# nju-websoft/OpenEA

Hardware: AMD Instinct MI355X
Metric: training triples/sec (k=10 truncated negatives + limited loss + Adagrad) (higher is better)
Workload: dtype f32; 1 GPU; BootEA/AlignE translational step, EN-FR-100K-V1 shape (synthetic), dim=100, GLOBAL batch=20000 positives (weak scaling: 20000 per GPU x 1 GPU), k=10, truncated eps=0.98; the same workload at every N (; global_batch=20000, entities=200000, parallelism=single

## Files before the change

openea_amd/csrc/step_plan.hip:

```cpp
#include <string.h>

#include <rocprim/rocprim.hpp>

#include <algorithm>

#include "common.h"
#include "step_plan.h"

namespace oea {

static size_t al256(size_t x) { return (x + 255) / 256 * 256; }
static int bits_for(uint64_t max_value) { int b = 1; while (b < 64 && (max_value >> b) != 0) ++b; return b; }

size_t step_plan_layout(int64_t n_total, int32_t steps, int64_t max_batch, int64_t n_ent, int32_t ld, void *base, StepPlanView *v) {
    const size_t m = (size_t)std::max<int64_t>(2 * n_total, 1);
    size_t off = 0;
    char *b = static_cast<char *>(base);
    auto take = [&](size_t bytes) { size_t o = off; off += al256(bytes); return b ? b + o : nullptr; };
    StepPlanView w{};
    w.keys_a = (uint64_t *)take(8 * m);
    w.keys_b = (uint64_t *)take(8 * m);
    w.vals_a = (uint32_t *)take(4 * m);
    w.vals_b = (uint32_t *)take(4 * m);
    w.ukeys = (uint64_t *)take(8 * m);
    w.ucount = (uint32_t *)take(4 * (m + 1));
    w.uoff = (uint32_t *)take(4 * (m + 1));
    w.n_unique = (int32_t *)take(4);
    w.step_first = (int32_t *)take(4 * ((size_t)steps + 1));
    w.pflags = (uint32_t *)take(4 * (size_t)std::max<int64_t>(n_total, 1));
    w.recs = (uint4 *)take(16 * m);
    w.inplan = (uint8_t *)take((size_t)std::max<int32_t>(steps, 1) * (size_t)n_ent);
    w.contrib = (float *)take(sizeof(float) * 2 * (size_t)std::max<int64_t>(max_batch, 1) * (size_t)ld);
    size_t t1 = 0, t2 = 0, t3 = 0;
    (void)rocprim::radix_sort_pairs(nullptr, t1, (const uint64_t *)nullptr, (uint64_t *)nullptr, (const uint32_t *)nullptr,
                                    (uint32_t *)nullptr, m, 0, 64, (hipStream_t)0);
    (void)rocprim::run_length_encode(nullptr, t2, (const uint64_t *)nullptr, m, (uint64_t *)nullptr, (uint32_t *)nullptr,
                                     (int32_t *)nullptr, (hipStream_t)0);
    (void)rocprim::exclusive_scan(nullptr, t3, (const uint32_t *)nullptr, (uint32_t *)nullptr, 0u, m + 1, rocprim::plus<uint32_t>(),
                                  (hipStream_t)0);
    const size_t n1 = (size_t)std::max<int64_t>(n_total, 1);
    w.temp_bytes = std::max(std::max(t1, std::max(t2, t3)), al256(4 * n1)) + 256;
    w.temp = take(w.temp_bytes);
    w.rel_order = (uint32_t *)take(4 * n1);
    w.row_bits = bits_for((uint64_t)std::max<int64_t>(n_ent - 1, 1));
    if (v) *v = w;
    return off;
}

namespace {

__global__ void plan_emit_kernel(const int32_t *__restrict__ pos_all, const int32_t *__restrict__ neg_all, int k,
                                 const int64_t *__restrict__ offsets, int steps, int64_t n_total, int row_bits,
                                 uint64_t *__restrict__ keys, uint32_t *__restrict__ vals) {
    const int64_t p = (int64_t)blockIdx.x * blockDim.x + threadIdx.x;
    if (p >= n_total) return;
    int lo = 0, hi = steps;
    while (hi - lo > 1) {
        const int mid = (lo + hi) >> 1;
        if (offsets[mid] <= p) lo = mid; else hi = mid;
    }
    const uint32_t pl = (uint32_t)(p - offsets[lo]);
    const int h = pos_all[3 * p], r = pos_all[3 * p + 1], t = pos_all[3 * p + 2];
    unsigned bad = 0, xh = 0, xt = 0;
    const int32_t *ng = neg_all + p * k * 3;
    for (int j = 0; j < k; ++j) {
        const unsigned a = (unsigned)(ng[3 * j] ^ h), b = (unsigned)(ng[3 * j + 2] ^ t), c = (unsigned)(ng[3 * j + 1] ^ r);
        bad |= c | min(a, b);
        xh |= a;
        xt |= b;
    }
    if (bad | min(xh, xt)) {
        keys[2 * p] = keys[2 * p + 1] = (uint64_t)steps << row_bits;
        vals[2 * p] = vals[2 * p + 1] = 0u;
        return;
    }
    const bool tails = xh == 0;
    const uint64_t sk = (uint64_t)lo << row_bits;
    keys[2 * p] = sk | (uint64_t)(uint32_t)h;
    vals[2 * p] = 2u * pl + (tails ? 0u : 1u);
    keys[2 * p + 1] = sk | (uint64_t)(uint32_t)t;
    vals[2 * p + 1] = 0x80000000u | (2u * pl + (tails ? 1u : 0u));
}

constexpr int kRelSortWaves = 8, kRelDigitBits = 10, kRelBins = 1 << kRelDigitBits, kRelAhead = 8;
__global__ __launch_bounds__(kRelSortWaves * 64) void plan_rel_order_kernel(const int32_t *__restrict__ pos_all, const int64_t *__restrict__ offsets,
                                                                            uint32_t *__restrict__ tmp, uint32_t *__restrict__ rel_order) {
    __shared__ uint32_t hist[kRelSortWaves][kRelBins];
    __shared__ uint32_t dbase[kRelBins];
    __shared__ uint32_t wsum[kRelSortWaves];
    __shared__ uint32_t rmax;
    const int64_t first = offsets[blockIdx.x];
    const uint32_t n = (uint32_t)(offsets[blockIdx.x + 1] - first);
    if (n == 0) return;
    const int32_t *rel = pos_all + 3 * first + 1;
    const uint32_t t = threadIdx.x, lane = t & 63u, w = t >> 6;
    const uint32_t slice = (n + kRelSortWaves - 1) / kRelSortWaves, c0 = min(w * slice, n), c1 = min(c0 + slice, n);
    const uint32_t groups = (c1 - c0 + 63u) / 64u;
    if (t == 0) rmax = 0u;
    int passes = 1;
    uint32_t *src = nullptr, *dst = nullptr;
    for (int pass = 0; pass < passes; ++pass) {
        const int shift = pass * kRelDigitBits;
        for (uint32_t i = t; i < kRelSortWaves * kRelBins; i += blockDim.x) (&hist[0][0])[i] = 0u;
        __syncthreads();
        uint32_t m = 0u;
        for (uint32_t g0 = 0; g0 < groups; g0 += kRelAhead) {
            uint32_t r[kRelAhead];
#pragma unroll
            for (int u = 0; u < kRelAhead; ++u) {
                const uint32_t i = c0 + (g0 + u) * 64u + lane;
                r[u] = i < c1 ? (uint32_t)rel[3 * (int64_t)(src ? src[i] : i)] : 0xffffffffu;
            }
#pragma unroll
            for (int u = 0; u < kRelAhead; ++u)
                if (c0 + (g0 + u) * 64u + lane < c1) {
                    m = max(m, r[u]);
                    atomicAdd(&hist[w][(r[u] >> shift) & (kRelBins - 1)], 1u);
                }
        }
        if (pass == 0) {
            for (int o = 32; o > 0; o >>= 1) m = max(m, (uint32_t)__shfl_xor((int)m, o));
            if (lane == 0) atomicMax(&rmax, m);
        }
        __syncthreads();
        if (pass == 0) {
            while (passes * kRelDigitBits < 32 && (rmax >> (passes * kRelDigitBits)) != 0u) ++passes;
            dst = (passes & 1) ? rel_order + first : tmp + first;
        }
        constexpr int DPT = kRelBins / (kRelSortWaves * 64);
        uint32_t tot[DPT], mine = 0u;
#pragma unroll
        for (int j = 0; j < DPT; ++j) {
            uint32_t run = 0u;
            for (int x = 0; x < kRelSortWaves; ++x) { const uint32_t c = hist[x][t * DPT + j]; hist[x][t * DPT + j] = run; run += c; }
            tot[j] = run;
            mine += run;
        }
        uint32_t inc = mine;
        for (int o = 1; o < 64; o <<= 1) { const uint32_t y = (uint32_t)__shfl_up((int)inc, o); if (lane >= (uint32_t)o) inc += y; }
        if (lane == 63u) wsum[w] = inc;
        __syncthreads();
        uint32_t before = inc - mine;
        for (uint32_t x = 0; x < w; ++x) before += wsum[x];
#pragma unroll
        for (int j = 0; j < DPT; ++j) { dbase[t * DPT + j] = before; before += tot[j]; }
        __syncthreads();
        for (uint32_t g0 = 0; g0 < groups; g0 += kRelAhead) {
            uint32_t idx[kRelAhead], dg[kRelAhead];
#pragma unroll
            for (int u = 0; u < kRelAhead; ++u) {
                const uint32_t i = c0 + (g0 + u) * 64u + lane;
                idx[u] = i < c1 ? (src ? src[i] : i) : 0u;
                dg[u] = i < c1 ? ((uint32_t)rel[3 * (int64_t)idx[u]] >> shift) & (kRelBins - 1) : 0u;
            }
#pragma unroll
            for (int u = 0; u < kRelAhead; ++u) {
                const bool on = c0 + (g0 + u) * 64u + lane < c1;
                const uint32_t d = dg[u];
                unsigned long long same = __ballot(on);
#pragma unroll
                for (int b = 0; b < kRelDigitBits; ++b) {
                    const unsigned long long has = __ballot(on && ((d >> b) & 1u));
                    same &= ((d >> b) & 1u) ? has : ~has;
                }
                if (on) {
                    const uint32_t rank = (uint32_t)__popcll(same & ((1ull << lane) - 1ull));
                    const uint32_t slot = hist[w][d] + dbase[d] + rank;
                    dst[slot] = idx[u];
                    __builtin_amdgcn_wave_barrier();
                    if (rank == 0u) hist[w][d] += (uint32_t)__popcll(same);
                }
                __builtin_amdgcn_wave_barrier();
            }
        }
        __threadfence_block();
        __syncthreads();
        src = dst;
        dst = (dst == tmp + first) ? rel_order + first : tmp + first;
    }
}

__global__ void plan_step_first_kernel(const uint64_t *__restrict__ ukeys, const int32_t *__restrict__ n_unique, int steps, int row_bits,
                                       int32_t *__restrict__ step_first) {
    const int s = blockIdx.x * blockDim.x + threadIdx.x;
    if (s > steps) return;
    const uint64_t key = (uint64_t)s << row_bits;
    int lo = 0, hi = *n_unique;
    while (lo < hi) {
        const int mid = (lo + hi) >> 1;
        if (ukeys[mid] < key) lo = mid + 1; else hi = mid;
    }
    step_first[s] = lo;
}

__global__ void plan_records_kernel(const uint64_t *__restrict__ ukeys, const uint32_t *__restrict__ uoff, const uint32_t *__restrict__ vals,
                                    const int32_t *__restrict__ n_unique, int steps, int row_bits, int64_t n_ent, uint4 *__restrict__ recs,
                                    uint8_t *__restrict__ inplan) {
    const int nu = *n_unique;
    for (int64_t i = (int64_t)blockIdx.x * blockDim.x + threadIdx.x; i < nu; i += (int64_t)gridDim.x * blockDim.x) {
        const uint64_t key = ukeys[i];
        const uint32_t row = (uint32_t)(key & (((uint64_t)1 << row_bits) - 1)), e0 = uoff[i], cnt = uoff[i + 1] - e0;
        recs[i] = make_uint4(row, e0, cnt, vals[e0]);
        const int64_t step = (int64_t)(key >> row_bits);
        if (step < steps && cnt <= kPlanHubEntries) inplan[step * n_ent + row] = 1;
    }
}

__global__ void plan_hub_kernel(const uint64_t *__restrict__ keys, const uint32_t *__restrict__ vals, int64_t m,
                                const int64_t *__restrict__ offsets, int steps, int row_bits, uint32_t *__restrict__ pflags) {
    const int64_t e = (int64_t)blockIdx.x * blockDim.x + threadIdx.x;
    if (e >= m) return;
    const uint64_t key = keys[e];
    const int64_t step = (int64_t)(key >> row_bits);
    if (step >= steps) return;
    int left = 0, right = 0;
    while (left < (int)kPlanHubEntries && e - left - 1 >= 0 && keys[e - left - 1] == key) ++left;
    while (left + right < (int)kPlanHubEntries && e + right + 1 < m && keys[e + right + 1] == key) ++right;
    if (left + right < (int)kPlanHubEntries) return;
    const uint32_t v = vals[e];
    atomicOr(&pflags[offsets[step] + ((v & 0x7fffffffu) >> 1)], (v >> 31) ? 2u : 1u);
}

__device__ __forceinline__ uint32_t mix32(uint32_t x) {
    x ^= x >> 16; x *= 0x7feb352du; x ^= x >> 15; x *= 0x846ca68bu; x ^= x >> 16;
    return x;
}
__device__ __forceinline__ uint32_t feistel_perm(uint32_t i, uint32_t n, int lbits, int rbits, const uint32_t (&key)[6]) {
    const uint32_t lmask = (1u << lbits) - 1u, rmask = (1u << rbits) - 1u;
    uint32_t x = i;
    do {
        uint32_t l = x >> rbits, r = x & rmask;
#pragma unroll
        for (int q = 0; q < 6; q += 2) {
            l = (l ^ mix32(r ^ key[q])) & lmask;
            r = (r ^ mix32(l ^ key[q + 1])) & rmask;
        }
        x = (l << rbits) | r;
    } while (x >= n);
    return x;
}
__global__ void layout_perm_kernel(const int32_t *__restrict__ triples, int64_t n1, int64_t n2, const int64_t *__restrict__ slot, int64_t n_slots,
                                   uint32_t k0, uint32_t k1, uint32_t epoch, int32_t *__restrict__ dall) {
    const int64_t j = (int64_t)blockIdx.x * blockDim.x + threadIdx.x;
    if (j >= n_slots) return;
    const int64_t sj = slot[j];
    const bool second = sj >= n1;
    const uint32_t n = (uint32_t)(second ? n2 : n1), i = (uint32_t)(second ? sj - n1 : sj);
    int bits = 1;
    while (bits < 32 && (1ull << bits) < (unsigned long long)n) ++bits;
    if (bits < 2) bits = 2;
    const int rbits = bits / 2, lbits = bits - rbits;
    const uint4 wa = philox4x32_10(epoch, second ? 1u : 0u, 0x5eedu, 0u, k0, k1), wb = philox4x32_10(epoch, second ? 1u : 0u, 0x5eedu, 1u, k0, k1);
    const uint32_t key[6] = {wa.x, wa.y, wa.z, wa.w, wb.x, wb.y};
    const int64_t src = (int64_t)feistel_perm(i, n, lbits, rbits, key) + (second ? n1 : 0);
    dall[3 * j] = triples[3 * src]; dall[3 * j + 1] = triples[3 * src + 1]; dall[3 * j + 2] = triples[3 * src + 2];
}

}
}

extern "C" {

size_t oea_step_plan_bytes(int64_t n_total, int32_t steps, int64_t max_batch, int64_t n_ent, int32_t ld) {
    if (n_total < 0 || steps < 0 || max_batch < 0 || n_ent <= 0 || ld <= 0) return 0;
    return oea::step_plan_layout(n_total, steps, max_batch, n_ent, ld, nullptr, nullptr);
}

int oea_step_plan_offsets(int64_t n_total, int32_t steps, int64_t max_batch, int64_t n_ent, int32_t ld, int64_t *out) {
    OEA_REQUIRE(out && n_total >= 0 && steps >= 0 && n_ent > 0 && ld > 0, "arguments");
    oea::StepPlanView v;
    char *base = reinterpret_cast<char *>(4096);
    const size_t total = oea::step_plan_layout(n_total, steps, max_batch, n_ent, ld, base, &v);
    out[0] = (char *)v.vals_b - base; out[1] = (char *)v.ukeys - base; out[2] = (char *)v.uoff - base;
    out[3] = (char *)v.n_unique - base; out[4] = (char *)v.step_first - base; out[5] = (char *)v.contrib - base;
    out[6] = v.row_bits; out[7] = (int64_t)total; out[8] = (char *)v.pflags - base;
    return OEA_OK;
}

int oea_step_plan_rel_order_offset(int64_t n_total, int32_t steps, int64_t max_batch, int64_t n_ent, int32_t ld, int64_t *out) {
    OEA_REQUIRE(out && n_total >= 0 && steps >= 0 && n_ent > 0 && ld > 0, "arguments");
    oea::StepPlanView v;
    char *base = reinterpret_cast<char *>(4096);
    (void)oea::step_plan_layout(n_total, steps, max_batch, n_ent, ld, base, &v);
    *out = (char *)v.rel_order - base;
    return OEA_OK;
}

size_t oea_epoch_layout_bytes(int64_t n) {
    return n < 0 ? 0 : 256;
}

int oea_epoch_layout(const int32_t *triples, int64_t n1, int64_t n2, const int64_t *slot, int64_t n_slots, uint64_t seed, uint32_t epoch,
                     int32_t *dall, void *workspace, size_t ws_bytes, void *stream) {
    OEA_REQUIRE(triples && (slot || n_slots == 0) && (dall || n_slots == 0), "null pointer");
    OEA_REQUIRE(n1 >= 0 && n2 >= 0 && n_slots >= 0 && n1 < ((int64_t)1 << 32) && n2 < ((int64_t)1 << 32), "sizes");
    (void)workspace; (void)ws_bytes;
    if (n1 + n2 == 0 || n_slots == 0) return OEA_OK;
    hipStream_t st = oea::as_stream(stream);
    oea::layout_perm_kernel<<<(unsigned)oea::ceil_div(n_slots, 256), 256, 0, st>>>(triples, n1, n2, slot, n_slots, (uint32_t)seed,
                                                                                   (uint32_t)(seed >> 32), epoch, dall);
    OEA_CHECK_HIP(hipGetLastError());
    return OEA_OK;
}

int oea_step_plan_build(const int32_t *pos_all, const int32_t *neg_all, int32_t k, const int64_t *offsets_dev, int64_t n_total,
                        int32_t steps, int64_t max_batch, int64_t n_ent, int32_t ld, void *plan, size_t plan_bytes, void *stream) {
    OEA_REQUIRE(pos_all && offsets_dev && plan && (neg_all || k == 0), "null pointer");
    OEA_REQUIRE(n_total >= 0 && steps >= 1 && k >= 0 && n_ent > 0 && ld > 0, "sizes");
    OEA_REQUIRE(2 * n_total < ((int64_t)1 << 31) && 2 * max_batch < ((int64_t)1 << 31), "entries and slots are 31-bit");
    oea::StepPlanView v;
    const size_t need = oea::step_plan_layout(n_total, steps, max_batch, n_ent, ld, plan, &v);
    OEA_REQUIRE(plan_bytes >= need, "plan workspace smaller than oea_step_plan_bytes");
    hipStream_t st = oea::as_stream(stream);
    const size_t m = (size_t)(2 * n_total);
    if (m == 0) {
        OEA_CHECK_HIP(hipMemsetAsync(v.n_unique, 0, sizeof(int32_t), st));
        OEA_CHECK_HIP(hipMemsetAsync(v.step_first, 0, sizeof(int32_t) * ((size_t)steps + 1), st));
        return OEA_OK;
    }
    oea::plan_rel_order_kernel<<<(unsigned)steps, oea::kRelSortWaves * 64, 0, st>>>(pos_all, offsets_dev, (uint32_t *)v.temp, v.rel_order);
    oea::plan_emit_kernel<<<(unsigned)oea::ceil_div(n_total, 256), 256, 0, st>>>(pos_all, neg_all, k, offsets_dev, steps, n_total, v.row_bits,
                                                                                 v.keys_a, v.vals_a);
    const int end_bit = std::min(64, v.row_bits + oea::bits_for((uint64_t)steps));
    size_t tb = v.temp_bytes;
    OEA_CHECK_HIP(rocprim::radix_sort_pairs(v.temp, tb, (const uint64_t *)v.keys_a, v.keys_b, (const uint32_t *)v.vals_a, v.vals_b, m, 0,
                                            (unsigned)end_bit, st));
    OEA_CHECK_HIP(hipMemsetAsync(v.ucount, 0, sizeof(uint32_t) * (m + 1), st));
    tb = v.temp_bytes;
    OEA_CHECK_HIP(rocprim::run_length_encode(v.temp, tb, (const uint64_t *)v.keys_b, m, v.ukeys, v.ucount, v.n_unique, st));
    tb = v.temp_bytes;
    OEA_CHECK_HIP(rocprim::exclusive_scan(v.temp, tb, (const uint32_t *)v.ucount, v.uoff, 0u, m + 1, rocprim::plus<uint32_t>(), st));
    oea::plan_step_first_kernel<<<(unsigned)oea::ceil_div(steps + 1, 256), 256, 0, st>>>(v.ukeys, v.n_unique, steps, v.row_bits, v.step_first);
    OEA_CHECK_HIP(hipMemsetAsync(v.pflags, 0, sizeof(uint32_t) * (size_t)n_total, st));
    OEA_CHECK_HIP(hipMemsetAsync(v.inplan, 0, (size_t)steps * (size_t)n_ent, st));
    oea::plan_records_kernel<<<(unsigned)std::min<int64_t>(oea::ceil_div((int64_t)m, 256), 4096), 256, 0, st>>>(
        v.ukeys, v.uoff, v.vals_b, v.n_unique, steps, v.row_bits, n_ent, v.recs, v.inplan);
    oea::plan_hub_kernel<<<(unsigned)oea::ceil_div((int64_t)m, 256), 256, 0, st>>>(v.keys_b, v.vals_b, (int64_t)m, offsets_dev, steps, v.row_bits,
                                                                                   v.pflags);
    OEA_CHECK_HIP(hipGetLastError());
    return OEA_OK;
}

}
```

Before: 292.7 million triples/s.

## Fuse step-plan post-sort into custom scan kernels and stage emit negatives in LDS

The chain of rocprim run_length_encode, exclusive_scan, step_first binary search, two memsets and the records and hub kernels is replaced by three custom kernels. A per-tile head count kernel (which also zeroes pflags and inplan), a decoupled scan kernel that writes unique keys, offsets, step_first and per-entry group indices, and a finish kernel that emits records and hub flags. The emit kernel stages negatives in shared memory, writes keys and values as vector stores, and skips the step binary search for rejected triples. The relation sort kernel doubles its waves and caches relation ids in 16-bit LDS to avoid re-gathering from global memory on later passes. The aim is fewer launches, fewer memsets and less global traffic in plan building, at the cost of more complex hand-written scan logic.

```diff
diff --git a/openea_amd/csrc/step_plan.hip b/openea_amd/csrc/step_plan.hip
--- a/openea_amd/csrc/step_plan.hip
+++ b/openea_amd/csrc/step_plan.hip
@@ -49,46 +49,65 @@
 
 namespace {
 
-__global__ void plan_emit_kernel(const int32_t *__restrict__ pos_all, const int32_t *__restrict__ neg_all, int k,
-                                 const int64_t *__restrict__ offsets, int steps, int64_t n_total, int row_bits,
-                                 uint64_t *__restrict__ keys, uint32_t *__restrict__ vals) {
-    const int64_t p = (int64_t)blockIdx.x * blockDim.x + threadIdx.x;
+constexpr int kEmitThreads = 256, kEmitStageBytes = 60 * 1024;
+template <bool STAGED>
+__global__ __launch_bounds__(kEmitThreads) void plan_emit_kernel(const int32_t *__restrict__ pos_all, const int32_t *__restrict__ neg_all, int k,
+                                                                 const int64_t *__restrict__ offsets, int steps, int64_t n_total, int row_bits,
+                                                                 uint64_t *__restrict__ keys, uint32_t *__restrict__ vals) {
+    extern __shared__ int4 emit_stage[];
+    const int32_t *stage = reinterpret_cast<const int32_t *>(emit_stage);
+    const int64_t pb = (int64_t)blockIdx.x * kEmitThreads, p = pb + threadIdx.x;
+    const int per = 3 * k;
+    if (STAGED) {
+        const int64_t cnt = min((int64_t)kEmitThreads, n_total - pb) * per, quads = cnt / 4;
+        const int32_t *src = neg_all + pb * per;
+        int32_t *st = reinterpret_cast<int32_t *>(emit_stage);
+        if ((reinterpret_cast<uintptr_t>(src) & 15u) == 0u) {
+            for (int64_t i = threadIdx.x; i < quads; i += kEmitThreads) emit_stage[i] = reinterpret_cast<const int4 *>(src)[i];
+            for (int64_t i = 4 * quads + threadIdx.x; i < cnt; i += kEmitThreads) st[i] = src[i];
+        } else {
+            for (int64_t i = threadIdx.x; i < cnt; i += kEmitThreads) st[i] = src[i];
+        }
+        __syncthreads();
+    }
     if (p >= n_total) return;
-    int lo = 0, hi = steps;
-    while (hi - lo > 1) {
-        const int mid = (lo + hi) >> 1;
-        if (offsets[mid] <= p) lo = mid; else hi = mid;
-    }
-    const uint32_t pl = (uint32_t)(p - offsets[lo]);
     const int h = pos_all[3 * p], r = pos_all[3 * p + 1], t = pos_all[3 * p + 2];
     unsigned bad = 0, xh = 0, xt = 0;
-    const int32_t *ng = neg_all + p * k * 3;
+    const int32_t *ng = STAGED ? stage + (int64_t)threadIdx.x * per : neg_all + p * per;
     for (int j = 0; j < k; ++j) {
         const unsigned a = (unsigned)(ng[3 * j] ^ h), b = (unsigned)(ng[3 * j + 2] ^ t), c = (unsigned)(ng[3 * j + 1] ^ r);
         bad |= c | min(a, b);
         xh |= a;
         xt |= b;
     }
+    ulonglong2 *key2 = reinterpret_cast<ulonglong2 *>(keys) + p;
+    uint2 *val2 = reinterpret_cast<uint2 *>(vals) + p;
     if (bad | min(xh, xt)) {
-        keys[2 * p] = keys[2 * p + 1] = (uint64_t)steps << row_bits;
-        vals[2 * p] = vals[2 * p + 1] = 0u;
+        const uint64_t sentinel = (uint64_t)steps << row_bits;
+        *key2 = make_ulonglong2(sentinel, sentinel);
+        *val2 = make_uint2(0u, 0u);
         return;
     }
+    int lo = 0, hi = steps;
+    while (hi - lo > 1) {
+        const int mid = (lo + hi) >> 1;
+        if (offsets[mid] <= p) lo = mid; else hi = mid;
+    }
+    const uint32_t pl = (uint32_t)(p - offsets[lo]);
     const bool tails = xh == 0;
     const uint64_t sk = (uint64_t)lo << row_bits;
-    keys[2 * p] = sk | (uint64_t)(uint32_t)h;
-    vals[2 * p] = 2u * pl + (tails ? 0u : 1u);
-    keys[2 * p + 1] = sk | (uint64_t)(uint32_t)t;
-    vals[2 * p + 1] = 0x80000000u | (2u * pl + (tails ? 1u : 0u));
-}
-
-constexpr int kRelSortWaves = 8, kRelDigitBits = 10, kRelBins = 1 << kRelDigitBits, kRelAhead = 8;
+    *key2 = make_ulonglong2(sk | (uint64_t)(uint32_t)h, sk | (uint64_t)(uint32_t)t);
+    *val2 = make_uint2(2u * pl + (tails ? 0u : 1u), 0x80000000u | (2u * pl + (tails ? 1u : 0u)));
+}
+
+constexpr int kRelSortWaves = 16, kRelDigitBits = 10, kRelBins = 1 << kRelDigitBits, kRelAhead = 8, kRelCache = 24 * 1024;
 __global__ __launch_bounds__(kRelSortWaves * 64) void plan_rel_order_kernel(const int32_t *__restrict__ pos_all, const int64_t *__restrict__ offsets,
                                                                             uint32_t *__restrict__ tmp, uint32_t *__restrict__ rel_order) {
     __shared__ uint32_t hist[kRelSortWaves][kRelBins];
     __shared__ uint32_t dbase[kRelBins];
     __shared__ uint32_t wsum[kRelSortWaves];
     __shared__ uint32_t rmax;
+    __shared__ uint16_t rcache[kRelCache];
     const int64_t first = offsets[blockIdx.x];
     const uint32_t n = (uint32_t)(offsets[blockIdx.x + 1] - first);
     if (n == 0) return;
@@ -98,6 +117,8 @@
     const uint32_t groups = (c1 - c0 + 63u) / 64u;
     if (t == 0) rmax = 0u;
     int passes = 1;
+    const bool fits = n <= (uint32_t)kRelCache;
+    bool cached = false;
     uint32_t *src = nullptr, *dst = nullptr;
     for (int pass = 0; pass < passes; ++pass) {
         const int shift = pass * kRelDigitBits;
@@ -109,7 +130,15 @@
 #pragma unroll
             for (int u = 0; u < kRelAhead; ++u) {
                 const uint32_t i = c0 + (g0 + u) * 64u + lane;
-                r[u] = i < c1 ? (uint32_t)rel[3 * (int64_t)(src ? src[i] : i)] : 0xffffffffu;
+                if (cached) r[u] = i < c1 ? (uint32_t)rcache[src[i]] : 0xffffffffu;
+                else r[u] = i < c1 ? (uint32_t)rel[3 * (int64_t)(src ? src[i] : i)] : 0xffffffffu;
+            }
+            if (pass == 0 && fits) {
+#pragma unroll
+                for (int u = 0; u < kRelAhead; ++u) {
+                    const uint32_t i = c0 + (g0 + u) * 64u + lane;
+                    if (i < c1) rcache[i] = (uint16_t)r[u];
+                }
             }
 #pragma unroll
             for (int u = 0; u < kRelAhead; ++u)
@@ -125,6 +154,7 @@
         __syncthreads();
         if (pass == 0) {
             while (passes * kRelDigitBits < 32 && (rmax >> (passes * kRelDigitBits)) != 0u) ++passes;
+            cached = fits && rmax <= 0xffffu;
             dst = (passes & 1) ? rel_order + first : tmp + first;
         }
         constexpr int DPT = kRelBins / (kRelSortWaves * 64);
@@ -151,7 +181,8 @@
             for (int u = 0; u < kRelAhead; ++u) {
                 const uint32_t i = c0 + (g0 + u) * 64u + lane;
                 idx[u] = i < c1 ? (src ? src[i] : i) : 0u;
-                dg[u] = i < c1 ? ((uint32_t)rel[3 * (int64_t)idx[u]] >> shift) & (kRelBins - 1) : 0u;
+                if (cached) dg[u] = i < c1 ? ((uint32_t)rcache[idx[u]] >> shift) & (kRelBins - 1) : 0u;
+                else dg[u] = i < c1 ? ((uint32_t)rel[3 * (int64_t)idx[u]] >> shift) & (kRelBins - 1) : 0u;
             }
 #pragma unroll
             for (int u = 0; u < kRelAhead; ++u) {
@@ -180,45 +211,130 @@
     }
 }
 
-__global__ void plan_step_first_kernel(const uint64_t *__restrict__ ukeys, const int32_t *__restrict__ n_unique, int steps, int row_bits,
-                                       int32_t *__restrict__ step_first) {
-    const int s = blockIdx.x * blockDim.x + threadIdx.x;
-    if (s > steps) return;
-    const uint64_t key = (uint64_t)s << row_bits;
-    int lo = 0, hi = *n_unique;
-    while (lo < hi) {
-        const int mid = (lo + hi) >> 1;
-        if (ukeys[mid] < key) lo = mid + 1; else hi = mid;
-    }
-    step_first[s] = lo;
-}
-
-__global__ void plan_records_kernel(const uint64_t *__restrict__ ukeys, const uint32_t *__restrict__ uoff, const uint32_t *__restrict__ vals,
-                                    const int32_t *__restrict__ n_unique, int steps, int row_bits, int64_t n_ent, uint4 *__restrict__ recs,
-                                    uint8_t *__restrict__ inplan) {
-    const int nu = *n_unique;
-    for (int64_t i = (int64_t)blockIdx.x * blockDim.x + threadIdx.x; i < nu; i += (int64_t)gridDim.x * blockDim.x) {
-        const uint64_t key = ukeys[i];
-        const uint32_t row = (uint32_t)(key & (((uint64_t)1 << row_bits) - 1)), e0 = uoff[i], cnt = uoff[i + 1] - e0;
-        recs[i] = make_uint4(row, e0, cnt, vals[e0]);
-        const int64_t step = (int64_t)(key >> row_bits);
-        if (step < steps && cnt <= kPlanHubEntries) inplan[step * n_ent + row] = 1;
-    }
-}
-
-__global__ void plan_hub_kernel(const uint64_t *__restrict__ keys, const uint32_t *__restrict__ vals, int64_t m,
-                                const int64_t *__restrict__ offsets, int steps, int row_bits, uint32_t *__restrict__ pflags) {
+constexpr int kScanThreads = 256, kScanPer = 8, kScanTile = kScanThreads * kScanPer;
+
+__device__ __forceinline__ uint32_t scan_block_sum(uint32_t x, uint32_t *sh) {
+    for (int o = 32; o > 0; o >>= 1) x += (uint32_t)__shfl_xor((int)x, o);
+    __syncthreads();
+    if ((threadIdx.x & 63u) == 0u) sh[threadIdx.x >> 6] = x;
+    __syncthreads();
+    uint32_t s = 0u;
+#pragma unroll
+    for (int w = 0; w < kScanThreads / 64; ++w) s += sh[w];
+    return s;
+}
+
+__global__ __launch_bounds__(kScanThreads) void plan_heads_kernel(const uint64_t *__restrict__ keys, int64_t m, uint32_t *__restrict__ tile_heads,
+                                                                  uint32_t *__restrict__ pflags, int64_t n_total, uint8_t *__restrict__ inplan,
+                                                                  int64_t inplan_bytes) {
+    __shared__ uint32_t sh[kScanThreads / 64];
+    const int64_t base = (int64_t)blockIdx.x * kScanTile;
+    uint32_t c = 0u;
+#pragma unroll
+    for (int j = 0; j < kScanPer; ++j) {
+        const int64_t e = base + j * kScanThreads + threadIdx.x;
+        if (e < m && (e == 0 || keys[e] != keys[e - 1])) ++c;
+    }
+    c = scan_block_sum(c, sh);
+    if (threadIdx.x == 0) tile_heads[blockIdx.x] = c;
+    const int64_t g = (int64_t)blockIdx.x * kScanThreads + threadIdx.x, gn = (int64_t)gridDim.x * kScanThreads;
+    const uint4 zero = make_uint4(0u, 0u, 0u, 0u);
+    const int64_t pq = n_total / 4, iq = inplan_bytes / 16;
+    for (int64_t i = g; i < pq; i += gn) reinterpret_cast<uint4 *>(pflags)[i] = zero;
+    for (int64_t i = 4 * pq + g; i < n_total; i += gn) pflags[i] = 0u;
+    for (int64_t i = g; i < iq; i += gn) reinterpret_cast<uint4 *>(inplan)[i] = zero;
+    for (int64_t i = 16 * iq + g; i < inplan_bytes; i += gn) inplan[i] = 0;
+}
+
+__global__ __launch_bounds__(kScanThreads) void plan_scan_kernel(const uint64_t *__restrict__ keys, int64_t m, const uint32_t *__restrict__ tile_heads,
+                                                                 int steps, int row_bits, uint64_t *__restrict__ ukeys, uint32_t *__restrict__ uoff,
+                                                                 int32_t *__restrict__ n_unique, int32_t *__restrict__ step_first,
+                                                                 uint32_t *__restrict__ eidx) {
+    __shared__ uint32_t sh[kScanThreads / 64];
+    const uint32_t t = threadIdx.x, lane = t & 63u, w = t >> 6;
+    const int64_t e0 = (int64_t)blockIdx.x * kScanTile + (int64_t)t * kScanPer;
+    uint64_t key[kScanPer], prev = 0u;
+    if (e0 + kScanPer <= m) {
+#pragma unroll
+        for (int j = 0; j < kScanPer; j += 2) {
+            const ulonglong2 q = *reinterpret_cast<const ulonglong2 *>(keys + e0 + j);
+            key[j] = q.x;
+            key[j + 1] = q.y;
+        }
+    } else {
+#pragma unroll
+        for (int j = 0; j < kScanPer; ++j) key[j] = e0 + j < m ? keys[e0 + j] : 0u;
+    }
+    if (e0 > 0 && e0 < m) prev = keys[e0 - 1];
+    uint32_t before = 0u, all = 0u;
+    for (uint32_t i = t; i < gridDim.x; i += kScanThreads) {
+        const uint32_t c = tile_heads[i];
+        all += c;
+        if (i < blockIdx.x) before += c;
+    }
+    before = scan_block_sum(before, sh);
+    all = scan_block_sum(all, sh);
+    if (blockIdx.x == 0 && t == 0) *n_unique = (int32_t)all;
+    uint32_t heads = 0u, mine = 0u;
+#pragma unroll
+    for (int j = 0; j < kScanPer; ++j) {
+        const int64_t e = e0 + j;
+        if (e < m && (e == 0 || key[j] != (j ? key[j - 1] : prev))) { heads |= 1u << j; ++mine; }
+    }
+    uint32_t inc = mine;
+    for (int o = 1; o < 64; o <<= 1) { const uint32_t y = (uint32_t)__shfl_up((int)inc, o); if (lane >= (uint32_t)o) inc += y; }
+    __syncthreads();
+    if (lane == 63u) sh[w] = inc;
+    __syncthreads();
+    uint32_t run = before + inc - mine;
+    for (uint32_t x = 0; x < w; ++x) run += sh[x];
+
+    uint32_t idx[kScanPer];
+#pragma unroll
+    for (int j = 0; j < kScanPer; ++j) {
+        const int64_t e = e0 + j;
+        if (e < m) {
+            const int st = min((int)(key[j] >> row_bits), steps);
+            if ((heads >> j) & 1u) {
+                ukeys[run] = key[j];
+                uoff[run] = (uint32_t)e;
+                const int ps = e == 0 ? -1 : (int)((j ? key[j - 1] : prev) >> row_bits);
+                for (int s = ps + 1; s <= st; ++s) step_first[s] = (int32_t)run;
+                ++run;
+            }
+            if (e >= (int64_t)all) uoff[e] = (uint32_t)m;
+            if (e == m - 1) {
+                uoff[m] = (uint32_t)m;
+                for (int s = st + 1; s <= steps; ++s) step_first[s] = (int32_t)all;
+            }
+        }
+        idx[j] = run - 1u;
+    }
+    if (e0 + kScanPer <= m) {
+#pragma unroll
+        for (int j = 0; j < kScanPer; j += 4) *reinterpret_cast<uint4 *>(eidx + e0 + j) = make_uint4(idx[j], idx[j + 1], idx[j + 2], idx[j + 3]);
+    } else {
+#pragma unroll
+        for (int j = 0; j < kScanPer; ++j) if (e0 + j < m) eidx[e0 + j] = idx[j];
+    }
+}
+
+__global__ __launch_bounds__(256) void plan_finish_kernel(const uint64_t *__restrict__ keys, const uint32_t *__restrict__ vals,
+                                                          const uint32_t *__restrict__ eidx, const uint32_t *__restrict__ uoff, int64_t m,
+                                                          const int64_t *__restrict__ offsets, int steps, int row_bits, int64_t n_ent,
+                                                          uint4 *__restrict__ recs, uint8_t *__restrict__ inplan, uint32_t *__restrict__ pflags) {
     const int64_t e = (int64_t)blockIdx.x * blockDim.x + threadIdx.x;
     if (e >= m) return;
+    const uint32_t i = eidx[e], first = uoff[i], cnt = uoff[i + 1] - first, v = vals[e];
     const uint64_t key = keys[e];
     const int64_t step = (int64_t)(key >> row_bits);
-    if (step >= steps) return;
-    int left = 0, right = 0;
-    while (left < (int)kPlanHubEntries && e - left - 1 >= 0 && keys[e - left - 1] == key) ++left;
-    while (left + right < (int)kPlanHubEntries && e + right + 1 < m && keys[e + right + 1] == key) ++right;
-    if (left + right < (int)kPlanHubEntries) return;
-    const uint32_t v = vals[e];
-    atomicOr(&pflags[offsets[step] + ((v & 0x7fffffffu) >> 1)], (v >> 31) ? 2u : 1u);
+    const bool listed = step < steps;
+    if ((int64_t)first == e) {
+        const uint32_t row = (uint32_t)(key & (((uint64_t)1 << row_bits) - 1));
+        recs[i] = make_uint4(row, first, cnt, v);
+        if (listed && cnt <= kPlanHubEntries) inplan[step * n_ent + row] = 1;
+    }
+    if (listed && cnt > kPlanHubEntries) atomicOr(&pflags[offsets[step] + ((v & 0x7fffffffu) >> 1)], (v >> 31) ? 2u : 1u);
 }
 
 __device__ __forceinline__ uint32_t mix32(uint32_t x) {
@@ -319,24 +435,26 @@
         return OEA_OK;
     }
     oea::plan_rel_order_kernel<<<(unsigned)steps, oea::kRelSortWaves * 64, 0, st>>>(pos_all, offsets_dev, (uint32_t *)v.temp, v.rel_order);
-    oea::plan_emit_kernel<<<(unsigned)oea::ceil_div(n_total, 256), 256, 0, st>>>(pos_all, neg_all, k, offsets_dev, steps, n_total, v.row_bits,
-                                                                                 v.keys_a, v.vals_a);
+    const unsigned emit_blocks = (unsigned)oea::ceil_div(n_total, oea::kEmitThreads);
+    const size_t stage_bytes = sizeof(int32_t) * 3 * (size_t)k * oea::kEmitThreads;
+    if (k > 0 && stage_bytes <= (size_t)oea::kEmitStageBytes)
+        oea::plan_emit_kernel<true><<<emit_blocks, oea::kEmitThreads, stage_bytes, st>>>(pos_all, neg_all, k, offsets_dev, steps, n_total, v.row_bits,
+                                                                                       v.keys_a, v.vals_a);
+    else
+        oea::plan_emit_kernel<false><<<emit_blocks, oea::kEmitThreads, 0, st>>>(pos_all, neg_all, k, offsets_dev, steps, n_total, v.row_bits,
+                                                                              v.keys_a, v.vals_a);
     const int end_bit = std::min(64, v.row_bits + oea::bits_for((uint64_t)steps));
     size_t tb = v.temp_bytes;
     OEA_CHECK_HIP(rocprim::radix_sort_pairs(v.temp, tb, (const uint64_t *)v.keys_a, v.keys_b, (const uint32_t *)v.vals_a, v.vals_b, m, 0,
                                             (unsigned)end_bit, st));
-    OEA_CHECK_HIP(hipMemsetAsync(v.ucount, 0, sizeof(uint32_t) * (m + 1), st));
-    tb = v.temp_bytes;
-    OEA_CHECK_HIP(rocprim::run_length_encode(v.temp, tb, (const uint64_t *)v.keys_b, m, v.ukeys, v.ucount, v.n_unique, st));
-    tb = v.temp_bytes;
-    OEA_CHECK_HIP(rocprim::exclusive_scan(v.temp, tb, (const uint32_t *)v.ucount, v.uoff, 0u, m + 1, rocprim::plus<uint32_t>(), st));
-    oea::plan_step_first_kernel<<<(unsigned)oea::ceil_div(steps + 1, 256), 256, 0, st>>>(v.ukeys, v.n_unique, steps, v.row_bits, v.step_first);
-    OEA_CHECK_HIP(hipMemsetAsync(v.pflags, 0, sizeof(uint32_t) * (size_t)n_total, st));
-    OEA_CHECK_HIP(hipMemsetAsync(v.inplan, 0, (size_t)steps * (size_t)n_ent, st));
-    oea::plan_records_kernel<<<(unsigned)std::min<int64_t>(oea::ceil_div((int64_t)m, 256), 4096), 256, 0, st>>>(
-        v.ukeys, v.uoff, v.vals_b, v.n_unique, steps, v.row_bits, n_ent, v.recs, v.inplan);
-    oea::plan_hub_kernel<<<(unsigned)oea::ceil_div((int64_t)m, 256), 256, 0, st>>>(v.keys_b, v.vals_b, (int64_t)m, offsets_dev, steps, v.row_bits,
-                                                                                   v.pflags);
+    const unsigned tiles = (unsigned)oea::ceil_div((int64_t)m, oea::kScanTile);
+    uint32_t *tile_heads = reinterpret_cast<uint32_t *>(v.keys_a), *eidx = v.vals_a;
+    oea::plan_heads_kernel<<<tiles, oea::kScanThreads, 0, st>>>(v.keys_b, (int64_t)m, tile_heads, v.pflags, n_total, v.inplan,
+                                                                (int64_t)steps * n_ent);
+    oea::plan_scan_kernel<<<tiles, oea::kScanThreads, 0, st>>>(v.keys_b, (int64_t)m, tile_heads, steps, v.row_bits, v.ukeys, v.uoff, v.n_unique,
+                                                               v.step_first, eidx);
+    oea::plan_finish_kernel<<<(unsigned)oea::ceil_div((int64_t)m, 256), 256, 0, st>>>(v.keys_b, v.vals_b, eidx, v.uoff, (int64_t)m, offsets_dev, steps,
+                                                                                      v.row_bits, n_ent, v.recs, v.inplan, v.pflags);
     OEA_CHECK_HIP(hipGetLastError());
     return OEA_OK;
 }
```

Result: no change. 293.2 million triples/s, median of 3 (+0.2%).
